# paolomandica/HALO

Hardware: AMD Instinct MI355X
Metric: acquisition-scored images/sec (1024x2048, C=256, 19 cls) (higher is better)
Workload: dtype f64

## Files before the change

### halo_amd/csrc/halo_score.hip

```cpp
#include "halo_common.hpp"
#include "halo_devmath.hpp"
#include "halo_select_plan.hpp"
#include "halo_softmax.hpp"
#include <stdlib.h>
#include <type_traits>

namespace halo {

constexpr int TPB = 256;
#ifndef HALO_FTPB
#define HALO_FTPB 128
#endif
#ifndef HALO_FEAT_WAVES
#define HALO_FEAT_WAVES 4
#endif
#ifndef HALO_FEAT_UNROLL
#define HALO_FEAT_UNROLL 8
#endif
#ifndef HALO_FEAT_STORE
#define HALO_FEAT_STORE 2
#endif
#ifndef HALO_FEAT_ENT_STORE
#define HALO_FEAT_ENT_STORE 1
#endif
#ifndef HALO_FEAT_LOGIT_NT
#define HALO_FEAT_LOGIT_NT 1
#endif
constexpr int FTPB = HALO_FTPB;

__device__ __forceinline__ double nan_min(double a, double b) { return (a != a) ? a : ((b != b) ? b : (b < a ? b : a)); }
__device__ __forceinline__ double nan_max(double a, double b) { return (a != a) ? a : ((b != b) ? b : (b > a ? b : a)); }

template <int NT = TPB>
__device__ __forceinline__ void block_minmax(double mn, double mx, double *out2)
{
    __shared__ double smn[NT / 64], smx[NT / 64];
// ... 877 lines not shown
}

__global__ void __launch_bounds__(TPB) k_box3_unc(const float *__restrict__ ent, int H, int W, int pk,
                                                  float *__restrict__ unc, double *__restrict__ partials)
{
    const int b = blockIdx.y;
    const long long hw = (long long)H * W;
    const long long i0 = ((long long)blockIdx.x * TPB + threadIdx.x) * 4;
    const bool live = i0 < hw;
    double mn = 0.0, mx = 0.0;
    const int y = live ? (int)(i0 / W) : 0, x = live ? (int)(i0 % W) : 0;
    float o[4];
    box3_row4(ent + (size_t)b * hw, H, W, y, x, live, pk, o);
    if (live) {
        if (unc) *reinterpret_cast<float4 *>(unc + (size_t)b * hw + i0) = make_float4(o[0], o[1], o[2], o[3]);
        mn = mx = (double)o[0];
#pragma unroll
        for (int j = 1; j < 4; ++j) { mn = nan_min(mn, (double)o[j]); mx = nan_max(mx, (double)o[j]); }
    }
    if (!partials) return;
    __shared__ double seed[2];
    if (threadIdx.x == 0) { seed[0] = mn; seed[1] = mx; }
    __syncthreads();
    if (!live) { mn = seed[0]; mx = seed[1]; }
    block_minmax<TPB>(mn, mx, partials + ((size_t)b * gridDim.x + blockIdx.x) * 2);
}

constexpr int BM_RPT = 4, BM_TW = 256, BM_TH = BM_RPT * (TPB / 64);

__device__ __forceinline__ float nan_minf(float a, float b) { return (a != a) ? a : ((b != b) ? b : (b < a ? b : a)); }
__device__ __forceinline__ float nan_maxf(float a, float b) { return (a != a) ? a : ((b != b) ? b : (b > a ? b : a)); }

__global__ void __launch_bounds__(TPB) k_box3_minmax(const float *__restrict__ ent, int H, int W, int pk, double *__restrict__ partials,
                                                     unsigned *__restrict__ hist_zero)
{
    const int b = blockIdx.z, lane = threadIdx.x & 63, wv = threadIdx.x >> 6;
    if (hist_zero) {
        const unsigned nb = gridDim.x * gridDim.y;
        for (unsigned l = blockIdx.y * gridDim.x + blockIdx.x; l < NB1 / TPB; l += nb) hist_zero[(size_t)b * NB1 + l * TPB + threadIdx.x] = 0u;
    }
    const int x = blockIdx.x * BM_TW + lane * 4, y0 = blockIdx.y * BM_TH + wv * BM_RPT;
    const float *ep = ent + (size_t)b * H * W;
    const bool xin = x < W;
    auto load_row = [&](int yy, float (&r)[6]) {
        const bool in = xin && yy >= 0 && yy < H;
        const float *row = ep + (size_t)(in ? yy : 0) * W;
        float4 q = make_float4(0.0f, 0.0f, 0.0f, 0.0f);
        if (in) q = *reinterpret_cast<const float4 *>(row + x);
        float left = lane_prev(q.w), right = lane_next(q.x);
        if (lane == 0) left = (in && x > 0) ? row[x - 1] : 0.0f;
        if (lane == 63) right = (in && x + 4 < W) ? row[x + 4] : 0.0f;
        r[0] = (in && x > 0) ? left : 0.0f;
        r[1] = q.x; r[2] = q.y; r[3] = q.z; r[4] = q.w;
        r[5] = (in && x + 4 < W) ? right : 0.0f;
    };
    float r0[6], r1[6], r2[6];
    load_row(y0 - 1, r0);
    load_row(y0, r1);
    float mn = 0.0f, mx = 0.0f;
    bool have = false;
#pragma unroll
    for (int k = 0; k < BM_RPT; ++k) {
        const int y = y0 + k;
        load_row(y + 1, r2);
        if (xin && y < H) {
#pragma unroll
            for (int j = 0; j < 4; ++j) {
                float a = 0.0f;
#pragma unroll
                for (int dx = 0; dx < 3; ++dx) a = a + r0[j + dx];
#pragma unroll
                for (int dx = 0; dx < 3; ++dx) a = a + r1[j + dx];
#pragma unroll
                for (int dx = 0; dx < 3; ++dx) a = a + r2[j + dx];
                const float o = box3_over_count(a, H, W, y, x + j, pk);
                if (!have) { mn = mx = o; have = true; }
                else { mn = nan_minf(mn, o); mx = nan_maxf(mx, o); }
            }
        }
#pragma unroll
        for (int q = 0; q < 6; ++q) { r0[q] = r1[q]; r1[q] = r2[q]; }
    }
    __shared__ float seedf[2];
    __shared__ float smn[TPB / 64], smx[TPB / 64];
    if (threadIdx.x == 0) { seedf[0] = mn; seedf[1] = mx; }
    __syncthreads();
    if (!have) { mn = seedf[0]; mx = seedf[1]; }
#pragma unroll
    for (int off = 32; off > 0; off >>= 1) {
        mn = nan_minf(mn, __shfl_xor(mn, off));
        mx = nan_maxf(mx, __shfl_xor(mx, off));
    }
    if (lane == 0) { smn[wv] = mn; smx[wv] = mx; }
    __syncthreads();
    if (threadIdx.x == 0) {
#pragma unroll
        for (int i = 1; i < TPB / 64; ++i) { mn = nan_minf(mn, smn[i]); mx = nan_maxf(mx, smx[i]); }
        double *out2 = partials + (((size_t)b * gridDim.y + blockIdx.y) * gridDim.x + blockIdx.x) * 2;
        out2[0] = (double)mn;
        out2[1] = (double)mx;
    }
}

__global__ void __launch_bounds__(TPB) k_minmax_f32(const float *__restrict__ x, long long hw,
                                                    double *__restrict__ partials)
{
    const int b = blockIdx.y;
    const long long i = (long long)blockIdx.x * TPB + threadIdx.x;
    const bool live = i < hw;
    double mn = 0.0, mx = 0.0;
    if (live) mn = mx = (double)x[(size_t)b * hw + i];
    __shared__ double seed[2];
    if (threadIdx.x == 0) { seed[0] = mn; seed[1] = mx; }
    __syncthreads();
    if (!live) { mn = seed[0]; mx = seed[1]; }
    block_minmax<TPB>(mn, mx, partials + ((size_t)b * gridDim.x + blockIdx.x) * 2);
}

__global__ void __launch_bounds__(TPB) k_fill_f32(float *__restrict__ x, long long n, float v)
{
    const long long i = (long long)blockIdx.x * TPB + threadIdx.x;
    if (i < n) x[i] = v;
}

template <typename TI>
__global__ void __launch_bounds__(TPB) k_combine(const TI *__restrict__ imp_raw, const float *__restrict__ unc_raw,
                                                 const double *__restrict__ stats, const unsigned char *__restrict__ active,
                                                 long long hw, int normalize, TI *__restrict__ score,
                                                 TI *__restrict__ imp_out, float *__restrict__ unc_out)
{
    const int b = blockIdx.y;
    const long long i = (long long)blockIdx.x * TPB + threadIdx.x;
    if (i >= hw) return;
    const size_t o = (size_t)b * hw + i;
    TI im = imp_raw[o];
    float un = unc_raw[o];
    if (normalize) {
        const float umn = (float)stats[b * 4 + 2], umx = (float)stats[b * 4 + 3];
        un = (un - umn) / (float)((double)umx - (double)umn);
        const TI imn = (TI)stats[b * 4 + 0], imx = (TI)stats[b * 4 + 1];
        if constexpr (sizeof(TI) == 8) im = (im - imn) / (imx - imn);
        else im = (im - imn) / (float)((double)imx - (double)imn);
    }
    TI s = im * (TI)un;
    if (active && active[o]) {
        if constexpr (sizeof(TI) == 8) s = __longlong_as_double(0xfff0000000000000ll);
        else s = __uint_as_float(0xff800000u);
    }
    score[o] = s;
    if (imp_out) imp_out[o] = im;
    if (unc_out) unc_out[o] = un;
}


constexpr int CB_ROWS = 16;

template <typename TI>
__global__ void __launch_bounds__(TPB) k_combine_box3(const TI *__restrict__ imp_raw, const float *__restrict__ ent,
                                                      const double *__restrict__ stats, const unsigned char *__restrict__ active,
                                                      int H, int W, int pk, int normalize, TI *__restrict__ score,
                                                      TI *__restrict__ imp_out, float *__restrict__ unc_out, SelHdr *__restrict__ rng,
                                                      unsigned *__restrict__ hist, int rows)
{
    __shared__ unsigned hl[NB1];
    const int b = blockIdx.z;
    const long long hw = (long long)H * W;
    const int x = (blockIdx.x * TPB + threadIdx.x) * 4;
    const bool live = x < W;
    float umn = 0.0f, uden = 1.0f;
    TI imn = (TI)0, iden = (TI)1;
    bool fin = false;
    if (normalize) {
        umn = (float)stats[b * 4 + 2];
        const float umx = (float)stats[b * 4 + 3];
        uden = (float)((double)umx - (double)umn);
        imn = (TI)stats[b * 4 + 0];
        const TI imx = (TI)stats[b * 4 + 1];
        if constexpr (sizeof(TI) == 8) iden = imx - imn;
        else iden = (float)((double)imx - (double)imn);
        fin = uden > 0.0f && uden < __builtin_inff() && iden > (TI)0 && iden < (TI)__builtin_inf();
        if (rng && blockIdx.x == 0 && blockIdx.y == 0 && threadIdx.x == 0) {
            SelHdr h;
            memset(&h, 0, sizeof(h));
            h.kmin_inv = ~order_key(0.0);
            h.kmax = order_key(1.0);
            h.nvalid = 1u;
            h.flags = fin ? (hist ? (unsigned)SEL_F_HIST : 0u) : (unsigned)SEL_F_BAD;
            rng[b] = h;
        }
    }
    const bool count = hist != nullptr && fin;
    if (count) {
        for (int j = threadIdx.x; j < NB1; j += TPB) hl[j] = 0u;
        __syncthreads();
    }
    ValRange vr;
    vr.lo = 0.0; vr.scale = (double)NB1; vr.ok = true;
    const int ybeg = blockIdx.y * rows, yend = ybeg + rows < H ? ybeg + rows : H;
    const float *ep = ent + (size_t)b * hw;
    const int lane = threadIdx.x & 63;
    struct RowRaw { float4 q; float el, er; bool in; };
    auto row_issue = [&](int yy) {
        RowRaw t;
        t.in = live && yy >= 0 && yy < H;
        const float *row = ep + (size_t)(t.in ? yy : 0) * W;
        t.q = make_float4(0.0f, 0.0f, 0.0f, 0.0f);
        t.el = 0.0f; t.er = 0.0f;
        if (t.in) t.q = *reinterpret_cast<const float4 *>(row + x);
        if (lane == 0 && t.in && x > 0) t.el = row[x - 1];
        if (lane == 63 && t.in && x + 4 < W) t.er = row[x + 4];
// ... 870 lines not shown
    float e[1];
    int pr[1];
    if (softmax_lean<O_T, 1>(p)) {
        finish_px<O_T, 1, true>(p, unc_type, pur_type, g, e, pr, pred != nullptr, ltab);
    } else {
        softmax_general<O_T, 1>(p);
        finish_px<O_T, 1, false>(p, unc_type, pur_type, g, e, pr, pred != nullptr);
    }
    ent[(size_t)b * hw + i] = e[0];
    if (pred) pred[(size_t)b * hw + i] = (short)pr[0];
}

__global__ void __launch_bounds__(TPB) k_logit_interp_lr(const float *__restrict__ logit, long long bstride, int O, int h, int w, int H,
                                                         int W, float sh, float sw, float *__restrict__ dst)
{
    const int b = blockIdx.y;
    const long long hw = (long long)H * W;
    const long long i = (long long)blockIdx.x * TPB + threadIdx.x;
    if (i >= hw) return;
    const int y = (int)(i / W), x = (int)(i % W);
    const Taps<float> ty = make_taps<float>(y, sh, h), tx = make_taps<float>(x, sw, w);
    const float *lb = logit + (size_t)b * bstride;
    for (int c = 0; c < O; ++c) {
        const float *pl = lb + (size_t)c * h * w;
        dst[((size_t)b * O + c) * hw + i] = bilerp<float>(pl[(size_t)ty.i0 * w + tx.i0], pl[(size_t)ty.i0 * w + tx.i1],
                                                          pl[(size_t)ty.i1 * w + tx.i0], pl[(size_t)ty.i1 * w + tx.i1], tx.l0, tx.l1, ty.l0, ty.l1);
    }
}

static inline bool aligned16(const void *p) { return ((uintptr_t)p & 15) == 0; }

struct FusedLogit { const float *logit; long long bstride; int O; int unc_type; float *ent; };

template <typename T, int VEC>
static void launch_feat(const T *feat, long long bstride, int C, long long hw, int B, int mode, double ks, double rks,
                        T *out, double *partials, int nblk, hipStream_t st, const FusedLogit *fl)
{
    dim3 grid(nblk, B), block(FTPB);
    constexpr int UNROLL = HALO_FEAT_UNROLL;
    unsigned xcd_g = 256;
    while (xcd_g > 1 && 8 * xcd_g > (unsigned)nblk) xcd_g >>= 1;
    if (8 * xcd_g > (unsigned)nblk) xcd_g = 0;
#define HALO_FEAT(M, FO_)                                                                                               \
    hipLaunchKernelGGL((k_feat_reduce<T, VEC, M, UNROLL, FO_>), grid, block, 0, st, feat, bstride, C, hw, ks, rks, out, \
                       partials, fl ? fl->logit : nullptr, fl ? fl->bstride : 0ll, fl ? fl->unc_type : 0, fl ? fl->ent : nullptr, \
                       xcd_g)
    const int fo = fl ? fl->O : 0;
    if (mode == 0) {
        if (fo == 19) HALO_FEAT(0, 19); else if (fo == 16) HALO_FEAT(0, 16); else HALO_FEAT(0, 0);
    } else {
        if (fo == 19) HALO_FEAT(1, 19); else if (fo == 16) HALO_FEAT(1, 16); else HALO_FEAT(1, 0);
    }
#undef HALO_FEAT
}

}

using namespace halo;

static_assert(RI_TW == LR_TW && RI_TH == LR_TH, "k_region_impurity3 writes one min/max partial per tile of the same shape");
static_assert(WB_TW % LR_TW == 0 && WB_TH % LR_TH == 0 && WH_TW % LR_TW == 0 && WH_TH % LR_TH == 0,
              "a wide-window tile is a union of whole 64 x 16 tiles: one partial per tile never needs more slots than those");
static size_t partial_slots(int64_t H, int64_t W)
{
    const size_t a = (size_t)cdiv(H * W, FTPB), b = (size_t)(cdiv(W, LR_TW) * cdiv(H, LR_TH));
    return a > b ? a : b;
}

extern "C" size_t halo_score_workspace_bytes(int64_t B, int64_t H, int64_t W)
{
    if (B <= 0 || H <= 0 || W <= 0) return 0;
    const size_t n = (size_t)B * H * W;
    const size_t nblk = partial_slots(H, W);
    size_t s = 0;
    s += align_up(n * 4, 256);
    s += align_up(n * 4, 256);
    s += align_up(n * 8, 256);
    s += align_up(n * 2, 256);
    s += 2 * align_up((size_t)B * nblk * 2 * 8, 256);
// ... 1 lines not shown
    return s + 1024;
}

extern "C" size_t halo_score_args_workspace_bytes(const halo_score_args *a)
{
    if (!a || a->struct_bytes != sizeof(halo_score_args)) return 0;
    size_t s = halo_score_workspace_bytes(a->B, a->H, a->W);
    if (s == 0 || a->route == HALO_SCORE_FULL) return s;
    if (a->route != HALO_SCORE_LR && a->route != HALO_SCORE_LR_GRAM) return 0;
    if (a->O <= 0) return 0;
    if (!(a->O == 19 || a->O == 16)) s += (size_t)a->B * a->O * a->H * a->W * 4 + 512;
    if (a->route == HALO_SCORE_LR) return s;
    if (a->hf <= 0 || a->wf <= 0) return 0;
    return s + (size_t)a->B * 5 * a->hf * a->wf * 8 + 512;
}

static inline bool reads_feat(int pur_type) { return pur_type == HALO_PUR_HYPER || pur_type == HALO_PUR_RADIUS || pur_type == HALO_PUR_EUC_NORM; }
static inline bool is_ripu(int pur_type) { return pur_type == HALO_PUR_RIPU || pur_type == HALO_PUR_ORACLE_RIPU; }
static inline void record(void *event, hipStream_t st) { if (event) (void)hipEventRecord((hipEvent_t)event, st); }

struct ScorePlan {
    float *ent, *unc_raw;
    double *imp_raw;
    short *pred;
    double *part_imp, *part_unc, *stats;
    float *lr_logit_full;
    double *gram;
    bool lr, need_feat, hist, f64out, fuse;
    int pad, normalize, mode;
    double ks, rks;
    long long hw;
    int nblk1, nblk_imp, nblk_unc;
    FusedLogit fl;
};

template <typename T>
static void lr_window(int out_size, int in_size, int tile, int &max_span)
{
    const T sc = out_size > 1 ? (T)(in_size - 1) / (T)(out_size - 1) : (T)0;
    max_span = 1;
    for (int o0 = 0; o0 < out_size; o0 += tile) {
        const int ol = o0 + tile - 1 < out_size ? o0 + tile - 1 : out_size - 1;
        T f = sc * (T)o0; int lo = (int)f; lo = lo > in_size - 1 ? in_size - 1 : lo;
        f = sc * (T)ol; int hi = (int)f; hi = hi > in_size - 1 ? in_size - 1 : hi; hi = hi + (hi < in_size - 1 ? 1 : 0);
        if (hi - lo + 1 > max_span) max_span = hi - lo + 1;
    }
}

template <typename T>
static int launch_feat_lr(const halo_score_args &a, ScorePlan &p, T *out, hipStream_t st)
{
    const T *feat = (const T *)a.feat;
    const long long bstride = a.feat_bstride;
    const int C = (int)a.C, hf = (int)a.hf, wf = (int)a.wf, H = (int)a.H, W = (int)a.W, B = (int)a.B, mode = p.mode;
    const double ks = p.ks, rks = p.rks;
    double *partials = p.part_imp;
    int &nblk = p.nblk_imp;
    int max_rows, max_cols;
    lr_window<T>(H, hf, LR_TH, max_rows);
    lr_window<T>(W, wf, LR_TW, max_cols);
    ++max_rows; ++max_cols;
    const T sh = H > 1 ? (T)(hf - 1) / (T)(H - 1) : (T)0, sw = W > 1 ? (T)(wf - 1) / (T)(W - 1) : (T)0;
    dim3 grid((unsigned)cdiv(W, LR_TW), (unsigned)cdiv(H, LR_TH), (unsigned)B), block(TPB);
    nblk = (int)(grid.x * grid.y);
    auto with_mode = [mode](auto launch) {
        if (mode == 0) launch(std::integral_constant<int, 0>());
        else launch(std::integral_constant<int, 1>());
    };
    if constexpr (sizeof(T) == 8) {
        const int units_per_ch = max_rows * ((max_cols + 2) / 2 + 1);
        int CCd = DMA_UNITS / units_per_ch;
        CCd = CCd > C ? C : CCd;
        const bool dma_ok = wf >= 2 && wf % 2 == 0 && bstride % 2 == 0 && aligned16(feat) && CCd >= 4;
        if (dma_ok) {
            const size_t lds = 2 * (size_t)DMA_UNITS * 16;
            const int need_rows = max_rows, need_u = (max_cols + 2) / 2;
            if ((double)sh <= 1.0 / 3.0 && H >= 2 * LR_TH) {
                int max_rows8;
                lr_window<T>(H, hf, 2 * LR_TH, max_rows8);
                ++max_rows8;
                dim3 grid8((unsigned)cdiv(W, LR_TW), (unsigned)cdiv(H, 2 * LR_TH), (unsigned)B);
#define HALO_LR_FIXED8(R_, U_)                                                                                                             \
                if (max_rows8 <= R_ && need_u <= U_) {                                                                                     \
                    nblk = (int)(grid8.x * grid8.y);                                                                                       \
                    with_mode([&](auto M) { hipLaunchKernelGGL((k_feat_reduce_lr_dmaf<decltype(M)::value, R_, U_, 2 * LR_PPT>), grid8, block, lds, st, \
                                                               (const double *)feat, bstride, C, hf, wf, H, W, (double)sh, (double)sw, ks, rks, (double *)out, partials); }); \
                    return HALO_OK;                                                                                                       \
                }
                HALO_LR_FIXED8(8, 8)
                HALO_LR_FIXED8(11, 10)
#undef HALO_LR_FIXED8
            }
#define HALO_LR_FIXED(R_, U_)                                                                                                              \
            if (need_rows <= R_ && need_u <= U_) {                                                                                         \
                with_mode([&](auto M) { hipLaunchKernelGGL((k_feat_reduce_lr_dmaf<decltype(M)::value, R_, U_>), grid, block, lds, st,      \
                                                           (const double *)feat, bstride, C, hf, wf, H, W, (double)sh, (double)sw, ks, rks, (double *)out, partials); }); \
                return HALO_OK;                                                                                                            \
            }
            HALO_LR_FIXED(6, 8)
            HALO_LR_FIXED(7, 10)
            HALO_LR_FIXED(8, 12)
#undef HALO_LR_FIXED
            with_mode([&](auto M) { hipLaunchKernelGGL((k_feat_reduce_lr_dma<decltype(M)::value>), grid, block, lds, st,
                                                       (const double *)feat, bstride, C, hf, wf, H, W, (double)sh, (double)sw, CCd, ks, rks, (double *)out, partials); });
            return HALO_OK;
        }
    }
    const size_t plane_bytes = (size_t)max_rows * max_cols * sizeof(T);
    if (plane_bytes > 48 * 1024) return fail(HALO_E_UNSUPPORTED, "halo_score: source window too large for LDS (downsampling?)");
    int CC = (int)((48 * 1024) / plane_bytes);
    CC = CC > (TPB / 64) * LR_STAGE_G ? (TPB / 64) * LR_STAGE_G : CC;
    CC = CC > C ? C : CC;
    const size_t lds = (size_t)CC * plane_bytes;
    with_mode([&](auto M) { hipLaunchKernelGGL((k_feat_reduce_lr<T, decltype(M)::value>), grid, block, lds, st,
                                               feat, bstride, C, hf, wf, H, W, sh, sw, max_rows, max_cols, CC, ks, rks, out, partials); });
    return HALO_OK;
}

static int check_padding(int pad, int k, int64_t H, int64_t W, const char *who)
{
    if (pad < HALO_PAD_ZEROS || pad > HALO_PAD_CIRCULAR) return fail(HALO_E_ARG, "%s: bad padding mode %d", who, pad);
    const int64_t r = k / 2, m = H < W ? H : W;
    if (pad == HALO_PAD_REFLECT && r >= m)
        return fail(HALO_E_ARG, "%s: padding_mode='reflect' needs the padding (%lld) to be smaller than the map (%lld x %lld)", who, (long long)r, (long long)H, (long long)W);
    if (pad == HALO_PAD_CIRCULAR && r > m)
        return fail(HALO_E_ARG, "%s: padding_mode='circular' needs the padding (%lld) to be at most the map size (%lld x %lld)", who, (long long)r, (long long)H, (long long)W);
    return HALO_OK;
}

static int check_score_args(const halo_score_args &a)
{
    if (a.struct_bytes != sizeof(halo_score_args))
        return fail(HALO_E_ARG, "halo_score: descriptor of %zu bytes, this library reads %zu (another ABI?)", a.struct_bytes, sizeof(halo_score_args));
    if (a.route < HALO_SCORE_FULL || a.route > HALO_SCORE_LR_GRAM) return fail(HALO_E_ARG, "halo_score: unknown route %d", a.route);
    const bool need_feat = reads_feat(a.pur_type);
    if (a.route != HALO_SCORE_FULL) {
        if (a.hl <= 0 || a.wl <= 0) return fail(HALO_E_ARG, "halo_score: bad low-res logit size");
        if (need_feat && (a.hf <= 0 || a.wf <= 0)) return fail(HALO_E_ARG, "halo_score: bad low-res embedding size");
    }
    if (a.route == HALO_SCORE_LR_GRAM && need_feat) {
        if (a.hf * a.wf > 0x7fffffffll) return fail(HALO_E_UNSUPPORTED, "halo_score: low-res planes of more than 2^31 elements (Gram route)");
        if (a.workspace_bytes < halo_score_args_workspace_bytes(&a)) return fail(HALO_E_WORKSPACE, "halo_score: workspace too small for the Gram route");
    }
    if (a.flags & ~(HALO_FLAG_NORMALIZE | (3 << 8))) return fail(HALO_E_ARG, "halo_score: unknown flag bits 0x%x", a.flags);
    if (!a.logit || !a.score || a.B <= 0 || a.O <= 0 || a.H <= 0 || a.W <= 0) return fail(HALO_E_ARG, "halo_score: null/empty argument");
    if (a.unc_type < 0 || a.unc_type > HALO_UNC_ZEROS) return fail(HALO_E_ARG, "halo_score: bad unc_type %d", a.unc_type);
    if (a.pur_type < 0 || a.pur_type > HALO_PUR_EUC_NORM) return fail(HALO_E_UNSUPPORTED, "Error: purity type '%d' not implemented", a.pur_type);
// ... 26 lines not shown

    Arena ar(a.workspace, a.workspace_bytes);
    p.ent = ar.take<float>(B * p.hw);
    p.unc_raw = ar.take<float>(B * p.hw);
    p.imp_raw = ar.take<double>(B * p.hw);
    p.pred = ar.take<short>(B * p.hw);
    p.part_imp = ar.take<double>(B * partial_slots(a.H, a.W) * 2);
    p.part_unc = ar.take<double>(B * partial_slots(a.H, a.W) * 2);
    p.stats = ar.take<double>(B * 4);
    p.lr_logit_full = (p.lr && !(a.O == 19 || a.O == 16)) ? ar.take<float>(B * a.O * p.hw) : nullptr;
    const bool gram_mode = a.route == HALO_SCORE_LR_GRAM && p.need_feat;
    if (gram_mode && a.feat_dtype != HALO_F64) return fail(HALO_E_UNSUPPORTED, "halo_score: float64 embeddings only on the Gram route");
    p.gram = gram_mode ? ar.take<double>(B * GRAM_MAPS * a.hf * a.wf) : nullptr;
    if (!ar.ok()) return fail(HALO_E_WORKSPACE, "halo_score: workspace too small");

    p.f64out = (a.pur_type == HALO_PUR_RADIUS || a.pur_type == HALO_PUR_EUC_NORM) && a.feat_dtype == HALO_F64;
    p.hist = is_ripu(a.pur_type) || a.pur_type == HALO_PUR_HYPER;
    p.mode = a.pur_type == HALO_PUR_EUC_NORM ? 1 : 0;
    p.ks = sqrt(fabs(-a.c) + 1e-15);
    p.rks = 1.0 / p.ks;

    const bool ent_only = (a.unc_type == HALO_UNC_ENTROPY || a.unc_type == HALO_UNC_PIXEL_ENTROPY) && !is_ripu(a.pur_type);
    const int fvec = !p.need_feat ? 0 : (a.feat_dtype == HALO_F64
        ? (((p.hw % 2 == 0) && (a.feat_bstride % 2 == 0) && aligned16(a.feat) && aligned16(p.imp_raw)) ? 2 : 1)
        : (((p.hw % 4 == 0) && (a.feat_bstride % 4 == 0) && aligned16(a.feat) && aligned16(p.imp_raw)) ? 4 : 1));
    p.fuse = !p.lr && p.need_feat && ent_only && (a.O == 19 || a.O == 16) && fvec > 1 && (a.logit_bstride % fvec == 0) &&
             (((uintptr_t)a.logit) % (4 * fvec) == 0);
    p.fl = FusedLogit{a.logit, (long long)a.logit_bstride, (int)a.O, a.unc_type, p.ent};
    return HALO_OK;
}

static void launch_logit_pass(const halo_score_args &a, const ScorePlan &p, hipStream_t st)
{
    if (p.fuse) return;
    const int B = (int)a.B, O = (int)a.O, H = (int)a.H, W = (int)a.W;
    const long long hw = p.hw, bstride = a.logit_bstride;
    const long long *gt = (const long long *)a.gt;
    short *pred = is_ripu(a.pur_type) ? p.pred : nullptr;
    const dim3 block(TPB), grid1((unsigned)p.nblk1, (unsigned)B);
    if (a.unc_type == HALO_UNC_ZEROS && !is_ripu(a.pur_type)) {
        hipLaunchKernelGGL(k_fill_f32, dim3((unsigned)cdiv(B * hw, TPB)), block, 0, st, p.ent, (long long)(B * hw), 0.0f);
    } else if (p.lr) {
        const int hl = (int)a.hl, wl = (int)a.wl;
        const float shl = H > 1 ? (float)(hl - 1) / (float)(H - 1) : 0.0f, swl = W > 1 ? (float)(wl - 1) / (float)(W - 1) : 0.0f;
        if (O == 19)
            hipLaunchKernelGGL((k_logit_maps_lr<19>), grid1, block, 0, st, a.logit, bstride, hl, wl, H, W, shl, swl, gt, a.unc_type, a.pur_type, p.ent, pred);
        else if (O == 16)
            hipLaunchKernelGGL((k_logit_maps_lr<16>), grid1, block, 0, st, a.logit, bstride, hl, wl, H, W, shl, swl, gt, a.unc_type, a.pur_type, p.ent, pred);
        else {
            hipLaunchKernelGGL(k_logit_interp_lr, grid1, block, 0, st, a.logit, bstride, O, hl, wl, H, W, shl, swl, p.lr_logit_full);
            hipLaunchKernelGGL(k_logit_maps_generic, grid1, block, 0, st, (const float *)p.lr_logit_full, (long long)(O * hw), gt, O, hw, a.unc_type, a.pur_type, 0, p.ent, pred);
        }
    } else {
        const bool vec4 = (hw % 4 == 0) && (bstride % 4 == 0) && aligned16(a.logit) && aligned16(p.ent);
        const dim3 grid4((unsigned)cdiv(hw, TPB * 4), (unsigned)B);
        if (O == 19 && vec4)
            hipLaunchKernelGGL((k_logit_maps<19, 4>), grid4, block, 0, st, a.logit, bstride, gt, hw, a.unc_type, a.pur_type, p.ent, pred);
        else if (O == 16 && vec4)
            hipLaunchKernelGGL((k_logit_maps<16, 4>), grid4, block, 0, st, a.logit, bstride, gt, hw, a.unc_type, a.pur_type, p.ent, pred);
        else
            hipLaunchKernelGGL(k_logit_maps_generic, grid1, block, 0, st, a.logit, bstride, gt, O, hw, a.unc_type, a.pur_type, 0, p.ent, pred);
    }
}

static void launch_gram(const halo_score_args &a, const ScorePlan &p, hipStream_t st)
{
    const double *feat = (const double *)a.feat;
    const long long bstride = a.feat_bstride;
    const int B = (int)a.B, C = (int)a.C, H = (int)a.H, W = (int)a.W, hf = (int)a.hf, wf = (int)a.wf;
    const dim3 block(TPB);
    const bool wide = wf >= 2 && wf % 2 == 0 && bstride % 2 == 0 && aligned16(feat) && aligned16(p.gram);
    if (wide) {
        const long long nwx = cdiv(wf, 128);
        int rows = 2;
        for (int cand = 8; cand > 2; cand >>= 1)
            if (B * nwx * cdiv(hf, cand) >= 1024) { rows = cand; break; }
        const long long nwaves = nwx * cdiv(hf, rows);
        const dim3 gg((unsigned)(cdiv(cdiv(nwaves, TPB / 64), 8) * 8), (unsigned)B);
#define HALO_GRAM2(U_, R_) hipLaunchKernelGGL((k_gram_lr2<U_, R_>), gg, block, 0, st, feat, bstride, C, hf, wf, p.gram)
        if (rows == 8) HALO_GRAM2(1, 8);
        else if (rows == 4) HALO_GRAM2(2, 4);
        else HALO_GRAM2(2, 2);
#undef HALO_GRAM2
    } else {
        const long long nwaves = cdiv(wf, GRAM_COLS) * cdiv(hf, 2);
        hipLaunchKernelGGL(k_gram_lr, dim3((unsigned)(cdiv(cdiv(nwaves, TPB / 64), 8) * 8), (unsigned)B), block, 0, st, feat, bstride, C, hf, wf, p.gram);
    }
    record(a.ev_feat_mid, st);
    const double shd = H > 1 ? (double)(hf - 1) / (double)(H - 1) : 0.0, swd = W > 1 ? (double)(wf - 1) / (double)(W - 1) : 0.0;
    const dim3 grid1((unsigned)p.nblk1, (unsigned)B);
    if (p.mode == 0) hipLaunchKernelGGL(k_radius_gram<0>, grid1, block, 0, st, p.gram, feat, bstride, C, hf, wf, H, W, shd, swd, p.ks, p.rks, p.imp_raw, p.part_imp);
    else hipLaunchKernelGGL(k_radius_gram<1>, grid1, block, 0, st, p.gram, feat, bstride, C, hf, wf, H, W, shd, swd, p.ks, p.rks, p.imp_raw, p.part_imp);
}

static int launch_feature_pass(const halo_score_args &a, ScorePlan &p, hipStream_t st)
{
    const int B = (int)a.B, C = (int)a.C;
    const long long hw = p.hw, bstride = a.feat_bstride;
    if (p.gram) {
        launch_gram(a, p, st);
        p.nblk_imp = p.nblk1;
    } else if (p.lr) {
        return a.feat_dtype == HALO_F64 ? launch_feat_lr<double>(a, p, p.imp_raw, st)
                                        : launch_feat_lr<float>(a, p, (float *)p.imp_raw, st);
    } else if (a.feat_dtype == HALO_F64) {
        const bool v2 = (hw % 2 == 0) && (bstride % 2 == 0) && aligned16(a.feat) && aligned16(p.imp_raw);
        p.nblk_imp = (int)cdiv(hw, v2 ? FTPB * 2 : FTPB);
        if (v2) launch_feat<double, 2>((const double *)a.feat, bstride, C, hw, B, p.mode, p.ks, p.rks, p.imp_raw, p.part_imp, p.nblk_imp, st, p.fuse ? &p.fl : nullptr);
        else launch_feat<double, 1>((const double *)a.feat, bstride, C, hw, B, p.mode, p.ks, p.rks, p.imp_raw, p.part_imp, p.nblk_imp, st, nullptr);
    } else {
        const bool v4 = (hw % 4 == 0) && (bstride % 4 == 0) && aligned16(a.feat) && aligned16(p.imp_raw);
        p.nblk_imp = (int)cdiv(hw, v4 ? FTPB * 4 : FTPB);
        if (v4) launch_feat<float, 4>((const float *)a.feat, bstride, C, hw, B, p.mode, p.ks, p.rks, (float *)p.imp_raw, p.part_imp, p.nblk_imp, st, p.fuse ? &p.fl : nullptr);
        else launch_feat<float, 1>((const float *)a.feat, bstride, C, hw, B, p.mode, p.ks, p.rks, (float *)p.imp_raw, p.part_imp, p.nblk_imp, st, nullptr);
    }
    return HALO_OK;
}

static int launch_tail(const halo_score_args &a, ScorePlan &p, hipStream_t st)
{
    const int64_t B = a.B, H = a.H, W = a.W;
    const long long hw = p.hw;
    const int normalize = p.normalize, box_pk = p.hist ? a.pksize : 0;
    const dim3 block(TPB), grid1((unsigned)p.nblk1, (unsigned)B);
    if (a.pur_type == HALO_PUR_HYPER) {
        hipLaunchKernelGGL(k_minmax_finalize, dim3((unsigned)B), block, 0, st, p.part_imp, p.nblk_imp, p.stats, 0);
        if (a.feat_dtype == HALO_F64) hipLaunchKernelGGL((k_quantize<double, short>), grid1, block, 0, st, (const double *)p.imp_raw, p.stats, hw, (int)a.K, p.pred);
        else hipLaunchKernelGGL((k_quantize<float, short>), grid1, block, 0, st, (const float *)p.imp_raw, p.stats, hw, (int)a.K, p.pred);
    }
    if (p.hist) {
        const float logK = (float)log((double)(a.pur_type == HALO_PUR_HYPER ? a.K : a.O));
        const int np = launch_region_impurity<short>((const short *)p.pred, B, H, W, a.pksize, a.pur_type == HALO_PUR_HYPER ? a.K : a.O, logK, (float *)p.imp_raw, (float *)nullptr, st,
                                                     normalize ? p.part_imp : nullptr, p.pad);
        p.nblk_imp = np ? np : p.nblk1;
        if (normalize && !np) hipLaunchKernelGGL(k_minmax_f32, grid1, block, 0, st, (const float *)p.imp_raw, hw, p.part_imp);
    } else if (a.pur_type == HALO_PUR_NONE) {
        hipLaunchKernelGGL(k_fill_f32, dim3((unsigned)cdiv(B * hw, TPB)), block, 0, st, (float *)p.imp_raw, (long long)(B * hw), 0.0f);
        if (normalize) hipLaunchKernelGGL(k_minmax_f32, grid1, block, 0, st, (const float *)p.imp_raw, hw, p.part_imp);
        p.nblk_imp = p.nblk1;
    }

    const int do_box = (a.unc_type == HALO_UNC_ENTROPY || a.unc_type == HALO_UNC_ORACLE_ACC) ? 1 : 0;
    const int box_route = do_box ? window_route(HALO_WINDOW_BOX, a.ksize, p.pad, 0, H, W) : 0;
    const bool box3 = box_route == 1 && aligned16(p.ent) && aligned16(p.unc_raw);
    const bool fuse_tail = box3 && B <= 65535 && H <= 65535 && aligned16(p.imp_raw) && aligned16(a.score) && (!a.impurity || aligned16(a.impurity)) &&
                           (!a.uncertainty || aligned16(a.uncertainty)) && (!a.active || ((uintptr_t)a.active & 3) == 0);
    SelHdr *rng_free = (a.score_range && normalize && fuse_tail) ? (SelHdr *)a.score_range : nullptr;
    unsigned *rng_hist = rng_free ? (unsigned *)((char *)a.score_range + range_hist_offset(B)) : nullptr;
    if (fuse_tail) {
        if (normalize) {
            const dim3 gridm((unsigned)cdiv(W, BM_TW), (unsigned)cdiv(H, BM_TH), (unsigned)B);
            p.nblk_unc = (int)(gridm.x * gridm.y);
            hipLaunchKernelGGL(k_box3_minmax, gridm, block, 0, st, (const float *)p.ent, (int)H, (int)W, box_pk, p.part_unc, rng_hist);
        }
    } else if (box3) {
        p.nblk_unc = (int)cdiv(hw, TPB * 4);
        hipLaunchKernelGGL(k_box3_unc, dim3((unsigned)p.nblk_unc, (unsigned)B), block, 0, st, (const float *)p.ent, (int)H, (int)W, box_pk, p.unc_raw,
                           normalize ? p.part_unc : nullptr);
    } else if (box_route == 2) {
        const dim3 gridw((unsigned)cdiv(W, WB_TW), (unsigned)cdiv(H, WB_TH), (unsigned)B);
        p.nblk_unc = (int)(gridw.x * gridw.y);
        hipLaunchKernelGGL(k_box_unc_tiled, gridw, block, 0, st, (const float *)p.ent, (int)H, (int)W, a.ksize, box_pk, p.unc_raw,
                           normalize ? p.part_unc : nullptr, p.pad);
    } else {
        hipLaunchKernelGGL(k_box_unc, grid1, block, 0, st, p.ent, (int)H, (int)W, a.ksize, do_box, box_pk, p.unc_raw, normalize ? p.part_unc : nullptr, p.pad);
    }

    if (normalize)
        hipLaunchKernelGGL(k_minmax_finalize2, dim3((unsigned)B, 2u), dim3(FIN_TPB), 0, st, (const double *)p.part_imp, p.nblk_imp,
                           (const double *)p.part_unc, p.nblk_unc, p.stats);
    if (fuse_tail) {
        int crows = CB_ROWS;
        while (crows > 1 && cdiv(W, TPB * 4) * cdiv(H, crows) * B < 1024) crows >>= 1;
        dim3 gridc((unsigned)cdiv(W, TPB * 4), (unsigned)cdiv(H, crows), (unsigned)B);
#define HALO_CB(T) hipLaunchKernelGGL((k_combine_box3<T>), gridc, block, 0, st, (const T *)p.imp_raw, (const float *)p.ent, p.stats, a.active, (int)H, (int)W, box_pk, normalize, (T *)a.score, (T *)a.impurity, a.uncertainty, rng_free, rng_hist, crows)
        if (p.f64out) HALO_CB(double);
        else HALO_CB(float);
#undef HALO_CB
    } else if (p.f64out) hipLaunchKernelGGL((k_combine<double>), grid1, block, 0, st, (const double *)p.imp_raw, p.unc_raw, p.stats, a.active, hw, normalize, (double *)a.score, (double *)a.impurity, a.uncertainty);
    else hipLaunchKernelGGL((k_combine<float>), grid1, block, 0, st, (const float *)p.imp_raw, p.unc_raw, p.stats, a.active, hw, normalize, (float *)a.score, (float *)a.impurity, a.uncertainty);
    if (a.score_range && !rng_free) {
        const int rc = score_range_exact(a.score, p.f64out ? HALO_F64 : HALO_F32, B, hw, a.score_range, st);
        if (rc != HALO_OK) return rc;
    }
    record(a.ev_tail_stop, st);
    return check_launch("halo_score");
}

static int score_impl(const halo_score_args &a, hipStream_t st)
{
    ScorePlan p;
    int rc = check_score_args(a);
    if (rc == HALO_OK) rc = make_score_plan(a, p);
    if (rc != HALO_OK) return rc;

    record(a.ev_logit_start, st);
    launch_logit_pass(a, p, st);
    record(a.ev_logit_stop, st);
    if (p.need_feat) {
        record(a.ev_feat_start, st);
        rc = launch_feature_pass(a, p, st);
        if (rc != HALO_OK) return rc;
        record(a.ev_feat_stop, st);
    }
    if (a.tail_stream && (hipStream_t)a.tail_stream != st) {
        if (!p.need_feat || !a.ev_feat_stop) return fail(HALO_E_ARG, "halo_score: a purity type that reads decoder_out and ev_feat_stop are required with a tail stream");
        if (hipStreamWaitEvent((hipStream_t)a.tail_stream, (hipEvent_t)a.ev_feat_stop, 0) != hipSuccess)
            return fail(HALO_E_LAUNCH, "halo_score: hipStreamWaitEvent: %s", hipGetErrorString(hipGetLastError()));
        st = (hipStream_t)a.tail_stream;
    }
    return launch_tail(a, p, st);
}

extern "C" int halo_score(const halo_score_args *a, void *stream)
{
    if (!a) return fail(HALO_E_ARG, "halo_score: null descriptor");
    return score_impl(*a, (hipStream_t)stream);
}

extern "C" int halo_region_uncertainty(const float *x, int64_t bstride, int is_prob, const int64_t *gt, int64_t B, int64_t O,
                                       int64_t H, int64_t W, int unc_type, int ksize, int do_box, float *out,
                                       void *workspace, size_t workspace_bytes, void *stream)
{
    hipStream_t st = (hipStream_t)stream;
    const int pad = (do_box >> 8) & 3;
    do_box &= 1;
    if (!x || !out || B <= 0 || O <= 0 || H <= 0 || W <= 0) return fail(HALO_E_ARG, "halo_region_uncertainty: null/empty argument");
    if (unc_type < 0 || unc_type > HALO_UNC_ZEROS) return fail(HALO_E_ARG, "halo_region_uncertainty: bad unc_type");
    if (unc_type == HALO_UNC_ORACLE_ACC && !gt) return fail(HALO_E_ARG, "halo_region_uncertainty: ground_truth required");
    if (ksize < 1 || !(ksize & 1)) return fail(HALO_E_ARG, "halo_region_uncertainty: window size must be odd");
    if (do_box) { const int rc = check_padding(pad, ksize, H, W, "halo_region_uncertainty"); if (rc != HALO_OK) return rc; }
    const long long hw = (long long)H * W;
    if (!workspace || workspace_bytes < (size_t)B * hw * 4 + 256) return fail(HALO_E_WORKSPACE, "halo_region_uncertainty: workspace too small");
    float *ent = (float *)(((uintptr_t)workspace + 255) & ~(uintptr_t)255);
    dim3 block(TPB), grid1((unsigned)cdiv(hw, TPB), (unsigned)B);
    float *dst = do_box ? ent : out;
// ... 62 lines not shown
```

Measured before the change: 1392.

## Fold min-max finalize into box3 and combine kernels; attach timing events to launches

Removes the separate k_minmax_finalize2 launch on the fused-tail path. k_box3_minmax now also pre-reduces the impurity partials into per-workgroup records, and k_combine_box3 reduces both record arrays in every block before writing stats. The box3 kernel issues all six row loads up front before the shuffles, so memory latency overlaps. Timing events are attached to kernel launches through hipExtLaunchKernelGGL instead of separate hipEventRecord calls. The trade is redundant per-block reduction work in the combine kernel, plus reuse of the unc_raw buffer as scratch.

```diff
diff --git a/halo_amd/csrc/halo_score.hip b/halo_amd/csrc/halo_score.hip
--- a/halo_amd/csrc/halo_score.hip
+++ b/halo_amd/csrc/halo_score.hip
@@ -2,6 +2,7 @@
 #include "halo_devmath.hpp"
 #include "halo_select_plan.hpp"
 #include "halo_softmax.hpp"
+#include <hip/hip_ext.h>
 #include <stdlib.h>
 #include <type_traits>
 
@@ -945,37 +946,59 @@
 __device__ __forceinline__ float nan_maxf(float a, float b) { return (a != a) ? a : ((b != b) ? b : (b > a ? b : a)); }
 
 __global__ void __launch_bounds__(TPB) k_box3_minmax(const float *__restrict__ ent, int H, int W, int pk, double *__restrict__ partials,
-                                                     unsigned *__restrict__ hist_zero)
+                                                     unsigned *__restrict__ hist_zero, const double *__restrict__ part_imp, int nblk_imp,
+                                                     double *__restrict__ rec_imp)
 {
     const int b = blockIdx.z, lane = threadIdx.x & 63, wv = threadIdx.x >> 6;
+    const unsigned nwg = gridDim.x * gridDim.y, wg = blockIdx.y * gridDim.x + blockIdx.x;
     if (hist_zero) {
-        const unsigned nb = gridDim.x * gridDim.y;
-        for (unsigned l = blockIdx.y * gridDim.x + blockIdx.x; l < NB1 / TPB; l += nb) hist_zero[(size_t)b * NB1 + l * TPB + threadIdx.x] = 0u;
+        for (unsigned l = wg; l < NB1 / TPB; l += nwg) hist_zero[(size_t)b * NB1 + l * TPB + threadIdx.x] = 0u;
+    }
+    double imn = 0.0, imx = 0.0;
+    if (rec_imp) {
+        const double2 *pi = reinterpret_cast<const double2 *>(part_imp) + (size_t)b * nblk_imp;
+        const int per = (int)(((unsigned)nblk_imp + nwg - 1u) / nwg);
+        const long long s0 = (long long)wg * per;
+        const long long s1 = s0 + per < (long long)nblk_imp ? s0 + per : (long long)nblk_imp;
+        const double2 p0 = pi[0];
+        imn = p0.x; imx = p0.y;
+        for (long long i = s0 + threadIdx.x; i < s1; i += TPB) { const double2 q = pi[i]; imn = nan_min(imn, q.x); imx = nan_max(imx, q.y); }
     }
     const int x = blockIdx.x * BM_TW + lane * 4, y0 = blockIdx.y * BM_TH + wv * BM_RPT;
     const float *ep = ent + (size_t)b * H * W;
     const bool xin = x < W;
-    auto load_row = [&](int yy, float (&r)[6]) {
-        const bool in = xin && yy >= 0 && yy < H;
-        const float *row = ep + (size_t)(in ? yy : 0) * W;
-        float4 q = make_float4(0.0f, 0.0f, 0.0f, 0.0f);
-        if (in) q = *reinterpret_cast<const float4 *>(row + x);
-        float left = lane_prev(q.w), right = lane_next(q.x);
-        if (lane == 0) left = (in && x > 0) ? row[x - 1] : 0.0f;
-        if (lane == 63) right = (in && x + 4 < W) ? row[x + 4] : 0.0f;
-        r[0] = (in && x > 0) ? left : 0.0f;
-        r[1] = q.x; r[2] = q.y; r[3] = q.z; r[4] = q.w;
-        r[5] = (in && x + 4 < W) ? right : 0.0f;
+    struct RowRaw { float4 q; float el, er; bool in; };
+    auto row_issue = [&](int yy) {
+        RowRaw t;
+        t.in = xin && yy >= 0 && yy < H;
+        const float *row = ep + (size_t)(t.in ? yy : 0) * W;
+        t.q = make_float4(0.0f, 0.0f, 0.0f, 0.0f);
+        t.el = 0.0f; t.er = 0.0f;
+        if (t.in) t.q = *reinterpret_cast<const float4 *>(row + x);
+        if (lane == 0 && t.in && x > 0) t.el = row[x - 1];
+        if (lane == 63 && t.in && x + 4 < W) t.er = row[x + 4];
+        return t;
     };
+    auto row_finish = [&](const RowRaw &t, float (&r)[6]) {
+        float left = lane_prev(t.q.w), right = lane_next(t.q.x);
+        if (lane == 0) left = t.el;
+        if (lane == 63) right = t.er;
+        r[0] = (t.in && x > 0) ? left : 0.0f;
+        r[1] = t.q.x; r[2] = t.q.y; r[3] = t.q.z; r[4] = t.q.w;
+        r[5] = (t.in && x + 4 < W) ? right : 0.0f;
+    };
+    RowRaw raw[BM_RPT + 2];
+#pragma unroll
+    for (int k = 0; k < BM_RPT + 2; ++k) raw[k] = row_issue(y0 - 1 + k);
     float r0[6], r1[6], r2[6];
-    load_row(y0 - 1, r0);
-    load_row(y0, r1);
+    row_finish(raw[0], r0);
+    row_finish(raw[1], r1);
     float mn = 0.0f, mx = 0.0f;
     bool have = false;
 #pragma unroll
     for (int k = 0; k < BM_RPT; ++k) {
         const int y = y0 + k;
-        load_row(y + 1, r2);
+        row_finish(raw[k + 2], r2);
         if (xin && y < H) {
 #pragma unroll
             for (int j = 0; j < 4; ++j) {
@@ -996,6 +1019,7 @@
     }
     __shared__ float seedf[2];
     __shared__ float smn[TPB / 64], smx[TPB / 64];
+    __shared__ double simn[TPB / 64], simx[TPB / 64];
     if (threadIdx.x == 0) { seedf[0] = mn; seedf[1] = mx; }
     __syncthreads();
     if (!have) { mn = seedf[0]; mx = seedf[1]; }
@@ -1004,14 +1028,25 @@
         mn = nan_minf(mn, __shfl_xor(mn, off));
         mx = nan_maxf(mx, __shfl_xor(mx, off));
     }
-    if (lane == 0) { smn[wv] = mn; smx[wv] = mx; }
+    if (rec_imp) {
+#pragma unroll
+        for (int off = 32; off > 0; off >>= 1) {
+            imn = nan_min(imn, __shfl_xor(imn, off));
+            imx = nan_max(imx, __shfl_xor(imx, off));
+        }
+    }
+    if (lane == 0) { smn[wv] = mn; smx[wv] = mx; simn[wv] = imn; simx[wv] = imx; }
     __syncthreads();
     if (threadIdx.x == 0) {
 #pragma unroll
         for (int i = 1; i < TPB / 64; ++i) { mn = nan_minf(mn, smn[i]); mx = nan_maxf(mx, smx[i]); }
-        double *out2 = partials + (((size_t)b * gridDim.y + blockIdx.y) * gridDim.x + blockIdx.x) * 2;
-        out2[0] = (double)mn;
-        out2[1] = (double)mx;
+        const size_t rec = (size_t)b * nwg + wg;
+        *reinterpret_cast<double2 *>(partials + rec * 2) = make_double2((double)mn, (double)mx);
+        if (rec_imp) {
+#pragma unroll
+            for (int i = 1; i < TPB / 64; ++i) { imn = nan_min(imn, simn[i]); imx = nan_max(imx, simx[i]); }
+            *reinterpret_cast<double2 *>(rec_imp + rec * 2) = make_double2(imn, imx);
+        }
     }
 }
 
@@ -1070,7 +1105,8 @@
 
 template <typename TI>
 __global__ void __launch_bounds__(TPB) k_combine_box3(const TI *__restrict__ imp_raw, const float *__restrict__ ent,
-                                                      const double *__restrict__ stats, const unsigned char *__restrict__ active,
+                                                      const double *__restrict__ rec_imp, const double *__restrict__ rec_unc, int nrec,
+                                                      double *__restrict__ stats, const unsigned char *__restrict__ active,
                                                       int H, int W, int pk, int normalize, TI *__restrict__ score,
                                                       TI *__restrict__ imp_out, float *__restrict__ unc_out, SelHdr *__restrict__ rng,
                                                       unsigned *__restrict__ hist, int rows)
@@ -1084,11 +1120,42 @@
     TI imn = (TI)0, iden = (TI)1;
     bool fin = false;
     if (normalize) {
-        umn = (float)stats[b * 4 + 2];
-        const float umx = (float)stats[b * 4 + 3];
+        __shared__ double sred[4][TPB / 64];
+        const double2 *ri = reinterpret_cast<const double2 *>(rec_imp) + (size_t)b * nrec;
+        const double2 *ru = reinterpret_cast<const double2 *>(rec_unc) + (size_t)b * nrec;
+        const double2 i0 = ri[0], u0 = ru[0];
+        double st4[4] = {i0.x, i0.y, u0.x, u0.y};
+        for (int i = threadIdx.x; i < nrec; i += TPB) {
+            const double2 qi = ri[i], qu = ru[i];
+            st4[0] = nan_min(st4[0], qi.x); st4[1] = nan_max(st4[1], qi.y);
+            st4[2] = nan_min(st4[2], qu.x); st4[3] = nan_max(st4[3], qu.y);
+        }
+#pragma unroll
+        for (int off = 32; off > 0; off >>= 1) {
+            st4[0] = nan_min(st4[0], __shfl_xor(st4[0], off)); st4[1] = nan_max(st4[1], __shfl_xor(st4[1], off));
+            st4[2] = nan_min(st4[2], __shfl_xor(st4[2], off)); st4[3] = nan_max(st4[3], __shfl_xor(st4[3], off));
+        }
+        if ((threadIdx.x & 63) == 0) {
+#pragma unroll
+            for (int k = 0; k < 4; ++k) sred[k][threadIdx.x >> 6] = st4[k];
+        }
+        __syncthreads();
+#pragma unroll
+        for (int k = 0; k < 4; ++k) st4[k] = sred[k][0];
+#pragma unroll
+        for (int w = 1; w < TPB / 64; ++w) {
+            st4[0] = nan_min(st4[0], sred[0][w]); st4[1] = nan_max(st4[1], sred[1][w]);
+            st4[2] = nan_min(st4[2], sred[2][w]); st4[3] = nan_max(st4[3], sred[3][w]);
+        }
+        if (blockIdx.x == 0 && blockIdx.y == 0 && threadIdx.x == 0) {
+#pragma unroll
+            for (int k = 0; k < 4; ++k) stats[b * 4 + k] = st4[k];
+        }
+        umn = (float)st4[2];
+        const float umx = (float)st4[3];
         uden = (float)((double)umx - (double)umn);
-        imn = (TI)stats[b * 4 + 0];
-        const TI imx = (TI)stats[b * 4 + 1];
+        imn = (TI)st4[0];
+        const TI imx = (TI)st4[1];
         if constexpr (sizeof(TI) == 8) iden = imx - imn;
         else iden = (float)((double)imx - (double)imn);
         fin = uden > 0.0f && uden < __builtin_inff() && iden > (TI)0 && iden < (TI)__builtin_inf();
@@ -2025,9 +2092,24 @@
 
 struct FusedLogit { const float *logit; long long bstride; int O; int unc_type; float *ent; };
 
+#ifndef HALO_EV_RIDE
+#define HALO_EV_RIDE 1
+#endif
+struct EvPair { void *start, *stop; };
+#define HALO_LAUNCH_EV(EV_, KERNEL_, GRID_, BLOCK_, LDS_, ST_, ...)                                                              \
+    do {                                                                                                                         \
+        if (HALO_EV_RIDE && ((EV_).start || (EV_).stop)) {                                                                       \
+            hipExtLaunchKernelGGL(KERNEL_, GRID_, BLOCK_, LDS_, ST_, (hipEvent_t)(EV_).start, (hipEvent_t)(EV_).stop, 0, __VA_ARGS__); \
+        } else {                                                                                                                 \
+            if ((EV_).start) (void)hipEventRecord((hipEvent_t)(EV_).start, ST_);                                                 \
+            hipLaunchKernelGGL(KERNEL_, GRID_, BLOCK_, LDS_, ST_, __VA_ARGS__);                                                  \
+            if ((EV_).stop) (void)hipEventRecord((hipEvent_t)(EV_).stop, ST_);                                                   \
+        }                                                                                                                        \
+    } while (0)
+
 template <typename T, int VEC>
 static void launch_feat(const T *feat, long long bstride, int C, long long hw, int B, int mode, double ks, double rks,
-                        T *out, double *partials, int nblk, hipStream_t st, const FusedLogit *fl)
+                        T *out, double *partials, int nblk, hipStream_t st, const FusedLogit *fl, EvPair ev = EvPair{nullptr, nullptr})
 {
     dim3 grid(nblk, B), block(FTPB);
     constexpr int UNROLL = HALO_FEAT_UNROLL;
@@ -2035,9 +2117,9 @@
     while (xcd_g > 1 && 8 * xcd_g > (unsigned)nblk) xcd_g >>= 1;
     if (8 * xcd_g > (unsigned)nblk) xcd_g = 0;
 #define HALO_FEAT(M, FO_)                                                                                               \
-    hipLaunchKernelGGL((k_feat_reduce<T, VEC, M, UNROLL, FO_>), grid, block, 0, st, feat, bstride, C, hw, ks, rks, out, \
-                       partials, fl ? fl->logit : nullptr, fl ? fl->bstride : 0ll, fl ? fl->unc_type : 0, fl ? fl->ent : nullptr, \
-                       xcd_g)
+    HALO_LAUNCH_EV(ev, (k_feat_reduce<T, VEC, M, UNROLL, FO_>), grid, block, 0, st, feat, bstride, C, hw, ks, rks, out, \
+                   partials, fl ? fl->logit : nullptr, fl ? fl->bstride : 0ll, fl ? fl->unc_type : 0, fl ? fl->ent : nullptr, \
+                   xcd_g)
     const int fo = fl ? fl->O : 0;
     if (mode == 0) {
         if (fo == 19) HALO_FEAT(0, 19); else if (fo == 16) HALO_FEAT(0, 16); else HALO_FEAT(0, 0);
@@ -2105,6 +2187,7 @@
     long long hw;
     int nblk1, nblk_imp, nblk_unc;
     FusedLogit fl;
+    EvPair ev_feat;
 };
 
 template <typename T>
@@ -2156,7 +2239,7 @@
 #define HALO_LR_FIXED8(R_, U_)                                                                                                             \
                 if (max_rows8 <= R_ && need_u <= U_) {                                                                                     \
                     nblk = (int)(grid8.x * grid8.y);                                                                                       \
-                    with_mode([&](auto M) { hipLaunchKernelGGL((k_feat_reduce_lr_dmaf<decltype(M)::value, R_, U_, 2 * LR_PPT>), grid8, block, lds, st, \
+                    with_mode([&](auto M) { HALO_LAUNCH_EV(p.ev_feat, (k_feat_reduce_lr_dmaf<decltype(M)::value, R_, U_, 2 * LR_PPT>), grid8, block, lds, st, \
                                                                (const double *)feat, bstride, C, hf, wf, H, W, (double)sh, (double)sw, ks, rks, (double *)out, partials); }); \
                     return HALO_OK;                                                                                                       \
                 }
@@ -2166,7 +2249,7 @@
             }
 #define HALO_LR_FIXED(R_, U_)                                                                                                              \
             if (need_rows <= R_ && need_u <= U_) {                                                                                         \
-                with_mode([&](auto M) { hipLaunchKernelGGL((k_feat_reduce_lr_dmaf<decltype(M)::value, R_, U_>), grid, block, lds, st,      \
+                with_mode([&](auto M) { HALO_LAUNCH_EV(p.ev_feat, (k_feat_reduce_lr_dmaf<decltype(M)::value, R_, U_>), grid, block, lds, st,      \
                                                            (const double *)feat, bstride, C, hf, wf, H, W, (double)sh, (double)sw, ks, rks, (double *)out, partials); }); \
                 return HALO_OK;                                                                                                            \
             }
@@ -2174,7 +2257,7 @@
             HALO_LR_FIXED(7, 10)
             HALO_LR_FIXED(8, 12)
 #undef HALO_LR_FIXED
-            with_mode([&](auto M) { hipLaunchKernelGGL((k_feat_reduce_lr_dma<decltype(M)::value>), grid, block, lds, st,
+            with_mode([&](auto M) { HALO_LAUNCH_EV(p.ev_feat, (k_feat_reduce_lr_dma<decltype(M)::value>), grid, block, lds, st,
                                                        (const double *)feat, bstride, C, hf, wf, H, W, (double)sh, (double)sw, CCd, ks, rks, (double *)out, partials); });
             return HALO_OK;
         }
@@ -2185,7 +2268,7 @@
     CC = CC > (TPB / 64) * LR_STAGE_G ? (TPB / 64) * LR_STAGE_G : CC;
     CC = CC > C ? C : CC;
     const size_t lds = (size_t)CC * plane_bytes;
-    with_mode([&](auto M) { hipLaunchKernelGGL((k_feat_reduce_lr<T, decltype(M)::value>), grid, block, lds, st,
+    with_mode([&](auto M) { HALO_LAUNCH_EV(p.ev_feat, (k_feat_reduce_lr<T, decltype(M)::value>), grid, block, lds, st,
                                                feat, bstride, C, hf, wf, H, W, sh, sw, max_rows, max_cols, CC, ks, rks, out, partials); });
     return HALO_OK;
 }
@@ -2278,21 +2361,25 @@
 
 static void launch_logit_pass(const halo_score_args &a, const ScorePlan &p, hipStream_t st)
 {
-    if (p.fuse) return;
+    const bool two_kernels = p.lr && !(a.unc_type == HALO_UNC_ZEROS && !is_ripu(a.pur_type)) && !(a.O == 19 || a.O == 16);
+    const bool ride = !p.fuse && !two_kernels;
+    const EvPair ev = ride ? EvPair{a.ev_logit_start, a.ev_logit_stop} : EvPair{nullptr, nullptr};
+    if (!ride) record(a.ev_logit_start, st);
+    if (p.fuse) { record(a.ev_logit_stop, st); return; }
     const int B = (int)a.B, O = (int)a.O, H = (int)a.H, W = (int)a.W;
     const long long hw = p.hw, bstride = a.logit_bstride;
     const long long *gt = (const long long *)a.gt;
     short *pred = is_ripu(a.pur_type) ? p.pred : nullptr;
     const dim3 block(TPB), grid1((unsigned)p.nblk1, (unsigned)B);
     if (a.unc_type == HALO_UNC_ZEROS && !is_ripu(a.pur_type)) {
-        hipLaunchKernelGGL(k_fill_f32, dim3((unsigned)cdiv(B * hw, TPB)), block, 0, st, p.ent, (long long)(B * hw), 0.0f);
+        HALO_LAUNCH_EV(ev, k_fill_f32, dim3((unsigned)cdiv(B * hw, TPB)), block, 0, st, p.ent, (long long)(B * hw), 0.0f);
     } else if (p.lr) {
         const int hl = (int)a.hl, wl = (int)a.wl;
         const float shl = H > 1 ? (float)(hl - 1) / (float)(H - 1) : 0.0f, swl = W > 1 ? (float)(wl - 1) / (float)(W - 1) : 0.0f;
         if (O == 19)
-            hipLaunchKernelGGL((k_logit_maps_lr<19>), grid1, block, 0, st, a.logit, bstride, hl, wl, H, W, shl, swl, gt, a.unc_type, a.pur_type, p.ent, pred);
+            HALO_LAUNCH_EV(ev, (k_logit_maps_lr<19>), grid1, block, 0, st, a.logit, bstride, hl, wl, H, W, shl, swl, gt, a.unc_type, a.pur_type, p.ent, pred);
         else if (O == 16)
-            hipLaunchKernelGGL((k_logit_maps_lr<16>), grid1, block, 0, st, a.logit, bstride, hl, wl, H, W, shl, swl, gt, a.unc_type, a.pur_type, p.ent, pred);
+            HALO_LAUNCH_EV(ev, (k_logit_maps_lr<16>), grid1, block, 0, st, a.logit, bstride, hl, wl, H, W, shl, swl, gt, a.unc_type, a.pur_type, p.ent, pred);
         else {
             hipLaunchKernelGGL(k_logit_interp_lr, grid1, block, 0, st, a.logit, bstride, O, hl, wl, H, W, shl, swl, p.lr_logit_full);
             hipLaunchKernelGGL(k_logit_maps_generic, grid1, block, 0, st, (const float *)p.lr_logit_full, (long long)(O * hw), gt, O, hw, a.unc_type, a.pur_type, 0, p.ent, pred);
@@ -2301,12 +2388,13 @@
         const bool vec4 = (hw % 4 == 0) && (bstride % 4 == 0) && aligned16(a.logit) && aligned16(p.ent);
         const dim3 grid4((unsigned)cdiv(hw, TPB * 4), (unsigned)B);
         if (O == 19 && vec4)
-            hipLaunchKernelGGL((k_logit_maps<19, 4>), grid4, block, 0, st, a.logit, bstride, gt, hw, a.unc_type, a.pur_type, p.ent, pred);
+            HALO_LAUNCH_EV(ev, (k_logit_maps<19, 4>), grid4, block, 0, st, a.logit, bstride, gt, hw, a.unc_type, a.pur_type, p.ent, pred);
         else if (O == 16 && vec4)
-            hipLaunchKernelGGL((k_logit_maps<16, 4>), grid4, block, 0, st, a.logit, bstride, gt, hw, a.unc_type, a.pur_type, p.ent, pred);
+            HALO_LAUNCH_EV(ev, (k_logit_maps<16, 4>), grid4, block, 0, st, a.logit, bstride, gt, hw, a.unc_type, a.pur_type, p.ent, pred);
         else
-            hipLaunchKernelGGL(k_logit_maps_generic, grid1, block, 0, st, a.logit, bstride, gt, O, hw, a.unc_type, a.pur_type, 0, p.ent, pred);
-    }
+            HALO_LAUNCH_EV(ev, k_logit_maps_generic, grid1, block, 0, st, a.logit, bstride, gt, O, hw, a.unc_type, a.pur_type, 0, p.ent, pred);
+    }
+    if (!ride) record(a.ev_logit_stop, st);
 }
 
 static void launch_gram(const halo_score_args &a, const ScorePlan &p, hipStream_t st)
@@ -2352,13 +2440,13 @@
     } else if (a.feat_dtype == HALO_F64) {
         const bool v2 = (hw % 2 == 0) && (bstride % 2 == 0) && aligned16(a.feat) && aligned16(p.imp_raw);
         p.nblk_imp = (int)cdiv(hw, v2 ? FTPB * 2 : FTPB);
-        if (v2) launch_feat<double, 2>((const double *)a.feat, bstride, C, hw, B, p.mode, p.ks, p.rks, p.imp_raw, p.part_imp, p.nblk_imp, st, p.fuse ? &p.fl : nullptr);
-        else launch_feat<double, 1>((const double *)a.feat, bstride, C, hw, B, p.mode, p.ks, p.rks, p.imp_raw, p.part_imp, p.nblk_imp, st, nullptr);
+        if (v2) launch_feat<double, 2>((const double *)a.feat, bstride, C, hw, B, p.mode, p.ks, p.rks, p.imp_raw, p.part_imp, p.nblk_imp, st, p.fuse ? &p.fl : nullptr, p.ev_feat);
+        else launch_feat<double, 1>((const double *)a.feat, bstride, C, hw, B, p.mode, p.ks, p.rks, p.imp_raw, p.part_imp, p.nblk_imp, st, nullptr, p.ev_feat);
     } else {
         const bool v4 = (hw % 4 == 0) && (bstride % 4 == 0) && aligned16(a.feat) && aligned16(p.imp_raw);
         p.nblk_imp = (int)cdiv(hw, v4 ? FTPB * 4 : FTPB);
-        if (v4) launch_feat<float, 4>((const float *)a.feat, bstride, C, hw, B, p.mode, p.ks, p.rks, (float *)p.imp_raw, p.part_imp, p.nblk_imp, st, p.fuse ? &p.fl : nullptr);
-        else launch_feat<float, 1>((const float *)a.feat, bstride, C, hw, B, p.mode, p.ks, p.rks, (float *)p.imp_raw, p.part_imp, p.nblk_imp, st, nullptr);
+        if (v4) launch_feat<float, 4>((const float *)a.feat, bstride, C, hw, B, p.mode, p.ks, p.rks, (float *)p.imp_raw, p.part_imp, p.nblk_imp, st, p.fuse ? &p.fl : nullptr, p.ev_feat);
+        else launch_feat<float, 1>((const float *)a.feat, bstride, C, hw, B, p.mode, p.ks, p.rks, (float *)p.imp_raw, p.part_imp, p.nblk_imp, st, nullptr, p.ev_feat);
     }
     return HALO_OK;
 }
@@ -2393,11 +2481,13 @@
                            (!a.uncertainty || aligned16(a.uncertainty)) && (!a.active || ((uintptr_t)a.active & 3) == 0);
     SelHdr *rng_free = (a.score_range && normalize && fuse_tail) ? (SelHdr *)a.score_range : nullptr;
     unsigned *rng_hist = rng_free ? (unsigned *)((char *)a.score_range + range_hist_offset(B)) : nullptr;
+    double *rec_imp = (double *)p.unc_raw;
     if (fuse_tail) {
         if (normalize) {
             const dim3 gridm((unsigned)cdiv(W, BM_TW), (unsigned)cdiv(H, BM_TH), (unsigned)B);
             p.nblk_unc = (int)(gridm.x * gridm.y);
-            hipLaunchKernelGGL(k_box3_minmax, gridm, block, 0, st, (const float *)p.ent, (int)H, (int)W, box_pk, p.part_unc, rng_hist);
+            hipLaunchKernelGGL(k_box3_minmax, gridm, block, 0, st, (const float *)p.ent, (int)H, (int)W, box_pk, p.part_unc, rng_hist,
+                               (const double *)p.part_imp, p.nblk_imp, rec_imp);
         }
     } else if (box3) {
         p.nblk_unc = (int)cdiv(hw, TPB * 4);
@@ -2412,14 +2502,14 @@
         hipLaunchKernelGGL(k_box_unc, grid1, block, 0, st, p.ent, (int)H, (int)W, a.ksize, do_box, box_pk, p.unc_raw, normalize ? p.part_unc : nullptr, p.pad);
     }
 
-    if (normalize)
+    if (normalize && !fuse_tail)
         hipLaunchKernelGGL(k_minmax_finalize2, dim3((unsigned)B, 2u), dim3(FIN_TPB), 0, st, (const double *)p.part_imp, p.nblk_imp,
                            (const double *)p.part_unc, p.nblk_unc, p.stats);
     if (fuse_tail) {
         int crows = CB_ROWS;
         while (crows > 1 && cdiv(W, TPB * 4) * cdiv(H, crows) * B < 1024) crows >>= 1;
         dim3 gridc((unsigned)cdiv(W, TPB * 4), (unsigned)cdiv(H, crows), (unsigned)B);
-#define HALO_CB(T) hipLaunchKernelGGL((k_combine_box3<T>), gridc, block, 0, st, (const T *)p.imp_raw, (const float *)p.ent, p.stats, a.active, (int)H, (int)W, box_pk, normalize, (T *)a.score, (T *)a.impurity, a.uncertainty, rng_free, rng_hist, crows)
+#define HALO_CB(T) hipLaunchKernelGGL((k_combine_box3<T>), gridc, block, 0, st, (const T *)p.imp_raw, (const float *)p.ent, (const double *)rec_imp, (const double *)p.part_unc, p.nblk_unc, p.stats, a.active, (int)H, (int)W, box_pk, normalize, (T *)a.score, (T *)a.impurity, a.uncertainty, rng_free, rng_hist, crows)
         if (p.f64out) HALO_CB(double);
         else HALO_CB(float);
 #undef HALO_CB
@@ -2440,14 +2530,14 @@
     if (rc == HALO_OK) rc = make_score_plan(a, p);
     if (rc != HALO_OK) return rc;
 
-    record(a.ev_logit_start, st);
     launch_logit_pass(a, p, st);
-    record(a.ev_logit_stop, st);
     if (p.need_feat) {
-        record(a.ev_feat_start, st);
+        const bool ride = !p.gram;
+        p.ev_feat = ride ? EvPair{a.ev_feat_start, a.ev_feat_stop} : EvPair{nullptr, nullptr};
+        if (!ride) record(a.ev_feat_start, st);
         rc = launch_feature_pass(a, p, st);
         if (rc != HALO_OK) return rc;
-        record(a.ev_feat_stop, st);
+        if (!ride) record(a.ev_feat_stop, st);
     }
     if (a.tail_stream && (hipStream_t)a.tail_stream != st) {
         if (!p.need_feat || !a.ev_feat_stop) return fail(HALO_E_ARG, "halo_score: a purity type that reads decoder_out and ev_feat_stop are required with a tail stream");
```

Result: no change. 1405, median of 6 (+0.9%).
